# MingyuKim87/Safe_Denoiser

Hardware: AMD Instinct MI355X
Metric: images/sec (512x512, 50 steps, SD-v1.4 + repellency) (higher is better)
Workload: dtype bf16; 1 GPU; README-default end to end (safree = svf = lra = true, safree_neg_prompt_config.json:26-28): token ids -> CLIP -> SAFREE projection -> DDPM 50 steps x UNet on 3 guidance branches with per-prompt text switching + safe_denoiser.yaml repellency (kernel_fast, M=515, sigma 3.15, scale .33, margin 1.6, window 780<=t<=1000) -> VAE decode -> uint8 512x512 images; SD-v1.4 UNet / CLIP / VAE with random weigh; guidance_branches=3, text_encoder_precision=bf16x3, prompts_per_batch=64, latent_repeat=3, renoise_draws_rank0=3520, parallelism=prompt-shard x1

## Files before the change

### safe_denoiser_amd/csrc/sdn_ffn.hip

```cpp
#include "sdn_gemm_common.h"

namespace sdn_gemm_detail {

#define SDN_STAMP(IDX) {}
#ifdef SDN_FFN_STAMPS
__device__ unsigned long long* g_ffn_stamps = nullptr;
#define SDN_FTS_DECL unsigned long long fts_prev = 0, fts_sum[8] = {0, 0, 0, 0, 0, 0, 0, 0};
#define SDN_FTS_MARK(I)                                                                         \
  {                                                                                             \
    unsigned long long t_;                                                                      \
    asm volatile("s_memtime %0\n\ts_waitcnt lgkmcnt(0)" : "=s"(t_)::"memory");                  \
    if ((I) >= 0) fts_sum[(I) < 0 ? 0 : (I)] += t_ - fts_prev;                                  \
    fts_prev = t_;                                                                              \
  }
#define SDN_FTS_FLUSH                                                                           \
  if (g_ffn_stamps && lane == 0)                                                                \
    for (int i_ = 0; i_ < 8; ++i_) g_ffn_stamps[((long)blockIdx.x * 8 + wid) * 8 + i_] = fts_sum[i_];
#else
#define SDN_FTS_DECL
#define SDN_FTS_MARK(I)
#define SDN_FTS_FLUSH
#endif

struct FfnArgs {
  const void* x;
  const float* stats;
  const void* w1;
  const float* c1; const float* d1;
  const void* w2;
  const float* b2;
  const void* residual;
  void* out;
  float* col_stats;
  int M;
};

#define SDN_FFN_CONTRACT(SA, SW)                                                                                           \
      {                                                                                                                    \
        typename T::v8 fa[2][4], fw[2][2];                                                                                 \
        _Pragma("unroll") for (int i = 0; i < 4; ++i)                                                                      \
          fa[0][i] = *reinterpret_cast<const typename T::v8*>((SA) + lds_off(i * 16 + fr, fq));                            \
        _Pragma("unroll") for (int j = 0; j < 2; ++j)                                                                      \
          fw[0][j] = *reinterpret_cast<const typename T::v8*>((SW) + lds_off(j * 16 + fr, fq));                            \
        _Pragma("unroll") for (int gi = 0; gi < 6; ++gi) {                                                                 \
          const int ks = gi / 3, g = gi % 3, nj = g == 2 ? 1 : 2;                                                          \
          if (gi + 1 < 6) {                                                                                                \
            const int ks1 = (gi + 1) / 3, g1 = (gi + 1) % 3, nj1 = g1 == 2 ? 1 : 2;                                        \
            _Pragma("unroll") for (int j = 0; j < nj1; ++j)                                                                \
              fw[(gi + 1) & 1][j] = *reinterpret_cast<const typename T::v8*>((SW) + lds_off((2 * g1 + j) * 16 + fr, ks1 * 4 + fq)); \
          }                                                                                                                \
          if (gi == 1) {                                                                                                   \
            _Pragma("unroll") for (int i = 0; i < 4; ++i)                                                                  \
              fa[1][i] = *reinterpret_cast<const typename T::v8*>((SA) + lds_off(i * 16 + fr, 4 + fq));                    \
          }                                                                                                                \
          __builtin_amdgcn_s_setprio(1);                                                                                   \
          _Pragma("unroll") for (int i = 0; i < 4; ++i)                                                                    \
            _Pragma("unroll") for (int j = 0; j < nj; ++j)                                                                 \
              acc[i][2 * g + j] = T::mfma16(fw[gi & 1][j], fa[ks][i], acc[i][2 * g + j]);                                  \
          __builtin_amdgcn_s_setprio(0);                                                                                   \
        }                                                                                                                  \
      }

template <typename T>
__global__ void __launch_bounds__(512, 1)
k_ffn320(const FfnArgs a) {
#if defined(__HIP_DEVICE_COMPILE__)
  constexpr int C = 320, HID = 4 * C, KT1 = C / BK, NCH = HID / 64, KT2 = NCH + KT1;
  constexpr int BM = 128, BN = C, THREADS = 512, NWAVES = 8, NREP = 5;
  constexpr int XIMG = BM * 128;
  constexpr int W2IMG = C * 128;
  constexpr int OFF_W2A = KT1 * XIMG;
  constexpr int OFF_RING = OFF_W2A + W2IMG;
  constexpr int LDS_BYTES = OFF_RING + W2IMG;
  constexpr unsigned OOB = 0x80000000u;
  __shared__ __attribute__((aligned(1024))) unsigned char smem[LDS_BYTES];

  const int tid = threadIdx.x, lane = tid & 63;
  const int wid = __builtin_amdgcn_readfirstlane(tid >> 6);
  SDN_FTS_DECL
  SDN_FTS_MARK(-1)
  const int wm = wid >> 2, wn = wid & 3;
  const int lrow = lane >> 3, lchunk = (lane & 7) ^ lrow;
  const int fr = lane & 15, fq = lane >> 4;
  const int m0 = blockIdx.x * BM, n0 = 0;

  const __amdgpu_buffer_rsrc_t rs_x = make_rsrc(a.x, (unsigned)((long)a.M * C * 2));
  const __amdgpu_buffer_rsrc_t rs_w1 = make_rsrc(a.w1, (unsigned)(2 * HID * C * 2));
  const __amdgpu_buffer_rsrc_t rs_w2 = make_rsrc(a.w2, (unsigned)(C * (HID + C) * 2));

#pragma unroll
  for (int q = 0; q < 10; ++q) {
    const int p = wid * 10 + q;
    const int kt = p >> 4, rg = p & 15;
    const int m = m0 + rg * 8 + lrow;
    const unsigned off = m < a.M ? (unsigned)(((long)m * C + kt * BK + lchunk * 8) * 2) : OOB;
    __builtin_amdgcn_raw_ptr_buffer_load_lds(rs_x, (lds_ptr_t)(smem + p * 1024), 16, off, 0, 0, 0);
  }
  const unsigned w1_lane = (unsigned)(((wid * 2 * 8 + lrow) * C + lchunk * 8) * 2);
  auto issue_w1 = [&](int g) {
    const int jc = g / KT1, kt = g - jc * KT1;
    unsigned char* dst = smem + OFF_RING + (g & 1) * XIMG + wid * 2048;
    const unsigned base = w1_lane + (unsigned)((jc * 128 * C + kt * BK) * 2);
    __builtin_amdgcn_raw_ptr_buffer_load_lds(rs_w1, (lds_ptr_t)dst, 16, base, 0, 0, 0);
    __builtin_amdgcn_raw_ptr_buffer_load_lds(rs_w1, (lds_ptr_t)(dst + 1024), 16, base + (unsigned)(8 * C * 2), 0, 0, 0);
  };
  const unsigned w2_lane = (unsigned)(((wid * 5 * 8 + lrow) * (HID + C) + lchunk * 8) * 2);
  auto issue_w2_slice = [&](int t, int q, int buf_off) {
    __builtin_amdgcn_raw_ptr_buffer_load_lds(rs_w2, (lds_ptr_t)(smem + buf_off + (wid * 5 + q) * 1024), 16,
                                             w2_lane + (unsigned)((q * 8 * (HID + C) + t * BK) * 2), 0, 0, 0);
  };

  issue_w1(0);
  f32x4 acc[4][NREP];
  {
    f32x4 bv[NREP];
#pragma unroll
    for (int j = 0; j < NREP; ++j) bv[j] = *reinterpret_cast<const f32x4*>(a.b2 + wn * 16 * NREP + j * 16 + fq * 4);
#pragma unroll
    for (int i = 0; i < 4; ++i)
#pragma unroll
      for (int j = 0; j < NREP; ++j) acc[i][j] = bv[j];
  }
  float ln_mu[4] = {0.f, 0.f, 0.f, 0.f}, ln_rs[4] = {0.f, 0.f, 0.f, 0.f};
  const bool own_stats = a.stats == nullptr;
  if (!own_stats) {
#pragma unroll
    for (int i = 0; i < 4; ++i) {
      const int m = m0 + wm * 64 + i * 16 + fr;
      const float2 st2 = *reinterpret_cast<const float2*>(a.stats + 2 * (long)(m < a.M ? m : 0));
      ln_mu[i] = st2.x; ln_rs[i] = st2.y;
    }
  }
  float ln_s1[4] = {0.f, 0.f, 0.f, 0.f}, ln_s2[4] = {0.f, 0.f, 0.f, 0.f};
  f32x4 cv[2], dv[2];
  auto load_cd = [&](int jc) {
#pragma unroll
    for (int j = 0; j < 2; ++j) {
      const int n = jc * 128 + wn * 32 + j * 16 + fq * 4;
      cv[j] = *reinterpret_cast<const f32x4*>(a.c1 + n); dv[j] = *reinterpret_cast<const f32x4*>(a.d1 + n);
    }
  };
  asm volatile("s_waitcnt vmcnt(0)" ::: "memory");
  __syncthreads();

  const unsigned char* sa_x = smem + (wm * 64) * 128;
  SDN_FTS_MARK(0)
  for (int jc = 0; jc < NCH; ++jc) {
    f32x4 acc1[4][2];
#pragma unroll
    for (int i = 0; i < 4; ++i) { acc1[i][0] = (f32x4){0.f, 0.f, 0.f, 0.f}; acc1[i][1] = (f32x4){0.f, 0.f, 0.f, 0.f}; }
#pragma unroll
    for (int kt = 0; kt < KT1; ++kt) {
      const int g = jc * KT1 + kt;
      if (kt == 0) load_cd(jc);
      if (g + 1 < NCH * KT1) issue_w1(g + 1);
      issue_w2_slice(jc, kt, OFF_W2A);
      const unsigned char* sa = sa_x + kt * XIMG;
      const unsigned char* sw = smem + OFF_RING + (g & 1) * XIMG + (wn * 32) * 128;
#pragma unroll
      for (int ks = 0; ks < 2; ++ks) {
        typename T::v8 fa[4], fw[2];
#pragma unroll
        for (int i = 0; i < 4; ++i) fa[i] = *reinterpret_cast<const typename T::v8*>(sa + lds_off(i * 16 + fr, ks * 4 + fq));
#pragma unroll
        for (int j = 0; j < 2; ++j) fw[j] = *reinterpret_cast<const typename T::v8*>(sw + lds_off(j * 16 + fr, ks * 4 + fq));
        if (own_stats && jc == 0) {
#pragma unroll
          for (int i = 0; i < 4; ++i) { ln_s1[i] = T::dot_ones(fa[i], ln_s1[i]); ln_s2[i] = T::dot_self(fa[i], ln_s2[i]); }
        }
        __builtin_amdgcn_s_setprio(1);
#pragma unroll
        for (int i = 0; i < 4; ++i)
#pragma unroll
          for (int j = 0; j < 2; ++j) acc1[i][j] = T::mfma16(fw[j], fa[i], acc1[i][j]);
        __builtin_amdgcn_s_setprio(0);
      }
      SDN_FTS_MARK(1)
      if (kt + 1 < KT1) asm volatile("s_waitcnt vmcnt(1)" ::: "memory");
      else asm volatile("s_waitcnt vmcnt(0)" ::: "memory");
      asm volatile("s_waitcnt lgkmcnt(0)" ::: "memory");
      SDN_FTS_MARK(2)
      __builtin_amdgcn_s_barrier();
      SDN_FTS_MARK(3)
    }
    if (own_stats && jc == 0) {
      const float invk = 1.0f / (float)C;
#pragma unroll
      for (int i = 0; i < 4; ++i) {
        float a1 = ln_s1[i], a2 = ln_s2[i];
        a1 += __shfl_xor(a1, 16, 64); a2 += __shfl_xor(a2, 16, 64);
        a1 += __shfl_xor(a1, 32, 64); a2 += __shfl_xor(a2, 32, 64);
        const float mu = a1 * invk;
        const float var = fmaxf(a2 * invk - mu * mu, 0.f);
        ln_mu[i] = mu; ln_rs[i] = __builtin_amdgcn_rsqf(var + 1e-5f);
      }
    }
    unsigned char* sh = smem + OFF_RING + ((jc * KT1 + KT1 - 1) & 1) * XIMG;
#pragma unroll
    for (int i = 0; i < 4; ++i) {
      const int row = wm * 64 + i * 16 + fr;
      const float mu = ln_mu[i], rs = ln_rs[i];
      const f32x4 hv = (acc1[i][0] - mu * cv[0]) * rs + dv[0], gv = (acc1[i][1] - mu * cv[1]) * rs + dv[1];
      uint2 pk;
      pk.x = T::pack2(hv[0] * gelu_erf(gv[0]), hv[1] * gelu_erf(gv[1]));
      pk.y = T::pack2(hv[2] * gelu_erf(gv[2]), hv[3] * gelu_erf(gv[3]));
      *reinterpret_cast<uint2*>(sh + lds_off(row, wn * 2 + (fq >> 1)) + (fq & 1) * 8) = pk;
    }
    SDN_FTS_MARK(4)
    __syncthreads();
    SDN_FTS_MARK(5)
    {
      const unsigned char* sa = sh + (wm * 64) * 128;
      const unsigned char* sw = smem + OFF_W2A + (wn * 16 * NREP) * 128;
      SDN_FFN_CONTRACT(sa, sw)
    }
    SDN_FTS_MARK(6)
    __syncthreads();
    SDN_FTS_MARK(5)
  }

  const __amdgpu_buffer_rsrc_t rs_res = make_rsrc(a.residual, (unsigned)((long)a.M * C * 2));
  auto issue_residual = [&](int img) {
#pragma unroll
    for (int q = 0; q < 2; ++q) {
      const int piece = img * 16 + wid * 2 + q;
      const int e = piece * 64 + lane;
      const int r = e / (BN / 8), c = e - r * (BN / 8);
      const int m = m0 + r;
      const unsigned off = m < a.M ? (unsigned)(((long)m * C + c * 8) * 2) : OOB;
      __builtin_amdgcn_raw_ptr_buffer_load_lds(rs_res, (lds_ptr_t)(smem + piece * 1024), 16, off, 0, 0, 0);
    }
  };
#pragma unroll
  for (int q = 0; q < 5; ++q) issue_w2_slice(NCH, q, OFF_W2A);
#pragma unroll
  for (int q = 0; q < 5; ++q) issue_w2_slice(NCH + 1, q, OFF_RING);
#pragma unroll
  for (int kt = 0; kt < KT1; ++kt) {
    const int boff = (kt & 1) ? OFF_RING : OFF_W2A;
    if (kt == 0) asm volatile("s_waitcnt vmcnt(5)" ::: "memory");
    else if (kt == 1) asm volatile("s_waitcnt vmcnt(7)" ::: "memory");
    else if (kt == 2 || kt == 3) asm volatile("s_waitcnt vmcnt(9)" ::: "memory");
    else asm volatile("s_waitcnt vmcnt(4)" ::: "memory");
    __builtin_amdgcn_s_barrier();
    {
      const unsigned char* sa = sa_x + kt * XIMG;
      const unsigned char* sw = smem + boff + (wn * 16 * NREP) * 128;
      SDN_FFN_CONTRACT(sa, sw)
    }
    asm volatile("s_waitcnt lgkmcnt(0)" ::: "memory");
    __builtin_amdgcn_s_barrier();
    if (kt + 2 < KT1) {
#pragma unroll
      for (int q = 0; q < 5; ++q) issue_w2_slice(NCH + kt + 2, q, boff);
    }
    issue_residual(kt);
  }
  asm volatile("s_waitcnt vmcnt(0)" ::: "memory");
  __syncthreads();

  GemmArgs g{};
  g.M = a.M; g.N = C; g.K = HID + C; g.ldc = C; g.n_valid = C; g.act = 0; g.out_kind = 0;
  g.residual = (const __bf16*)a.residual; g.out = a.out; g.col_stats = a.col_stats; g.res_lds = 1;
  g.res_bytes = (unsigned)((long)a.M * C * 2); g.rows_per_batch = 0; g.residual_bcast = 0;
  constexpr int LNF = 0, WGM = 2, NSTAGE = 2, STAGE = LDS_BYTES / 2;
  constexpr int CW_PAD = (BN + 8) * 2;
  const bool staged = true;
  const int out_cols = BN;
  const bool res_lds = true;
  const int CW = BN * 2;
  const bool lean = true, lean_gelu = false, lean_gate = false, lean_erf = false;
  constexpr int PASSES = 1, WM_PER_PASS = WGM / PASSES, ROWS_PER_PASS = 64 * WM_PER_PASS;
  static_assert(BM * CW_PAD <= NSTAGE * STAGE - 8 * BN * 8, "staged tile and the column-sum scratch must fit the LDS");
#define SDN_EPI_RES_PRELOADED
#define SDN_PASS 0
#include "sdn_gemm_epilogue.inc"
#undef SDN_PASS
#undef SDN_EPI_RES_PRELOADED
  SDN_FTS_MARK(7)
  SDN_FTS_FLUSH
  (void)NWAVES; (void)WGM; (void)lean_gelu; (void)lean_gate; (void)lean_erf; (void)staged; (void)CW_PAD; (void)KT2;
#endif
}

}
using namespace sdn_gemm_detail;

#ifdef SDN_FFN_STAMPS
extern "C" int sdn_debug_set_ffn_stamps(void* p) { return (int)hipMemcpyToSymbol(HIP_SYMBOL(sdn_gemm_detail::g_ffn_stamps), &p, sizeof(p)); }
#endif
extern "C" int sdn_ffn_geglu_fused(int32_t dtype, int64_t M, int32_t C, const void* x, const float* row_stats, const void* w1_folded, const float* c1,
                        const float* d1, const void* w_cat, const float* b_cat, const void* residual, void* out, float* col_stats,
                        void* stream) {
  auto al16 = [](const void* p) { return (reinterpret_cast<uintptr_t>(p) & 15) == 0; };
  if (dtype < 0 || dtype > 1 || C != 320 || M < 0 || !x || !w1_folded || !c1 || !d1 || !w_cat || !b_cat || !residual || !out)
    return SDN_E_INVALID;
  if (!al16(x) || !al16(w1_folded) || !al16(c1) || !al16(d1) || !al16(w_cat) || !al16(b_cat) || !al16(residual) || !al16(out) ||
      (reinterpret_cast<uintptr_t>(row_stats) & 7) || (reinterpret_cast<uintptr_t>(col_stats) & 7))
    return SDN_E_INVALID;
  if (M * C * 2 >= (1L << 31)) return SDN_E_INVALID;
  if (M == 0) return SDN_OK;
  FfnArgs a{x, row_stats, w1_folded, c1, d1, w_cat, b_cat, residual, out, col_stats, (int)M};
  const unsigned grid = (unsigned)((M + 127) / 128);
  record_gemm_launch(4, dtype, 10, 2, 2, row_stats ? 2 : 1, (int)grid, 1, 1, 0);
  if (dtype == 1) hipLaunchKernelGGL((k_ffn320<SdnF16>), dim3(grid), dim3(512), 0, (hipStream_t)stream, a);
  else hipLaunchKernelGGL((k_ffn320<SdnBF16>), dim3(grid), dim3(512), 0, (hipStream_t)stream, a);
  return sdn_launch_status();
}
```

Before: 8.340 images/sec.

## Stream W1 and W2 chunks through a unified 4-stage LDS ring in fused FFN

New measurement: 8.441 images/sec (median of 6 runs). 1.2% higher.

```diff
diff --git a/safe_denoiser_amd/csrc/sdn_ffn.hip b/safe_denoiser_amd/csrc/sdn_ffn.hip
--- a/safe_denoiser_amd/csrc/sdn_ffn.hip
+++ b/safe_denoiser_amd/csrc/sdn_ffn.hip
@@ -69,9 +69,12 @@
   constexpr int BM = 128, BN = C, THREADS = 512, NWAVES = 8, NREP = 5;
   constexpr int XIMG = BM * 128;
   constexpr int W2IMG = C * 128;
-  constexpr int OFF_W2A = KT1 * XIMG;
-  constexpr int OFF_RING = OFF_W2A + W2IMG;
-  constexpr int LDS_BYTES = OFF_RING + W2IMG;
+  constexpr int NSLOT = 8, NRING = 4;
+  constexpr int OFF_RING = KT1 * XIMG;
+  constexpr int OFF_H = OFF_RING + NRING * XIMG;
+  constexpr int OFF_TA = OFF_RING, OFF_TB = OFF_RING + W2IMG;
+  constexpr int LDS_BYTES = OFF_H + XIMG;
+  static_assert(OFF_TB + W2IMG == LDS_BYTES && NSLOT % NRING == 0, "ring + H = the tail's two weight buffers; stage = slot & 3");
   constexpr unsigned OOB = 0x80000000u;
   __shared__ __attribute__((aligned(1024))) unsigned char smem[LDS_BYTES];
 
@@ -97,12 +100,23 @@
     __builtin_amdgcn_raw_ptr_buffer_load_lds(rs_x, (lds_ptr_t)(smem + p * 1024), 16, off, 0, 0, 0);
   }
   const unsigned w1_lane = (unsigned)(((wid * 2 * 8 + lrow) * C + lchunk * 8) * 2);
-  auto issue_w1 = [&](int g) {
-    const int jc = g / KT1, kt = g - jc * KT1;
-    unsigned char* dst = smem + OFF_RING + (g & 1) * XIMG + wid * 2048;
-    const unsigned base = w1_lane + (unsigned)((jc * 128 * C + kt * BK) * 2);
-    __builtin_amdgcn_raw_ptr_buffer_load_lds(rs_w1, (lds_ptr_t)dst, 16, base, 0, 0, 0);
-    __builtin_amdgcn_raw_ptr_buffer_load_lds(rs_w1, (lds_ptr_t)(dst + 1024), 16, base + (unsigned)(8 * C * 2), 0, 0, 0);
+  const unsigned w2ab_lane = (unsigned)((((wid >> 1) * 16 * NREP + (wid & 1) * 16 + lrow) * (HID + C) + lchunk * 8) * 2);
+  const unsigned w2c_lane = (unsigned)((((wid >> 1) * 16 * NREP + 64 + (wid & 1) * 8 + lrow) * (HID + C) + lchunk * 8) * 2);
+  auto issue_slot = [&](int jc, int u) {
+    if (u >= NSLOT) { u -= NSLOT; ++jc; }
+    if (jc >= NCH) return;
+    unsigned char* stage = smem + OFF_RING + (u & (NRING - 1)) * XIMG;
+    if (u < KT1) {
+      const unsigned base = w1_lane + (unsigned)((jc * 128 * C + u * BK) * 2);
+      __builtin_amdgcn_raw_ptr_buffer_load_lds(rs_w1, (lds_ptr_t)(stage + wid * 2048), 16, base, 0, 0, 0);
+      __builtin_amdgcn_raw_ptr_buffer_load_lds(rs_w1, (lds_ptr_t)(stage + wid * 2048 + 1024), 16, base + (unsigned)(8 * C * 2), 0, 0, 0);
+    } else if (u < NSLOT - 1) {
+      const unsigned base = w2ab_lane + (unsigned)(((u - KT1) * 32 * (HID + C) + jc * BK) * 2);
+      __builtin_amdgcn_raw_ptr_buffer_load_lds(rs_w2, (lds_ptr_t)(stage + wid * 2048), 16, base, 0, 0, 0);
+      __builtin_amdgcn_raw_ptr_buffer_load_lds(rs_w2, (lds_ptr_t)(stage + wid * 2048 + 1024), 16, base + (unsigned)(8 * (HID + C) * 2), 0, 0, 0);
+    } else {
+      __builtin_amdgcn_raw_ptr_buffer_load_lds(rs_w2, (lds_ptr_t)(stage + wid * 1024), 16, w2c_lane + (unsigned)(jc * BK * 2), 0, 0, 0);
+    }
   };
   const unsigned w2_lane = (unsigned)(((wid * 5 * 8 + lrow) * (HID + C) + lchunk * 8) * 2);
   auto issue_w2_slice = [&](int t, int q, int buf_off) {
@@ -110,7 +124,7 @@
                                              w2_lane + (unsigned)((q * 8 * (HID + C) + t * BK) * 2), 0, 0, 0);
   };
 
-  issue_w1(0);
+  issue_slot(0, 0); issue_slot(0, 1); issue_slot(0, 2);
   f32x4 acc[4][NREP];
   {
     f32x4 bv[NREP];
@@ -146,17 +160,16 @@
   const unsigned char* sa_x = smem + (wm * 64) * 128;
   SDN_FTS_MARK(0)
   for (int jc = 0; jc < NCH; ++jc) {
+    const bool last = jc == NCH - 1;
     f32x4 acc1[4][2];
 #pragma unroll
     for (int i = 0; i < 4; ++i) { acc1[i][0] = (f32x4){0.f, 0.f, 0.f, 0.f}; acc1[i][1] = (f32x4){0.f, 0.f, 0.f, 0.f}; }
 #pragma unroll
     for (int kt = 0; kt < KT1; ++kt) {
-      const int g = jc * KT1 + kt;
       if (kt == 0) load_cd(jc);
-      if (g + 1 < NCH * KT1) issue_w1(g + 1);
-      issue_w2_slice(jc, kt, OFF_W2A);
+      issue_slot(jc, kt + 3);
       const unsigned char* sa = sa_x + kt * XIMG;
-      const unsigned char* sw = smem + OFF_RING + (g & 1) * XIMG + (wn * 32) * 128;
+      const unsigned char* sw = smem + OFF_RING + (kt & (NRING - 1)) * XIMG + (wn * 32) * 128;
 #pragma unroll
       for (int ks = 0; ks < 2; ++ks) {
         typename T::v8 fa[4], fw[2];
@@ -176,13 +189,15 @@
         __builtin_amdgcn_s_setprio(0);
       }
       SDN_FTS_MARK(1)
-      if (kt + 1 < KT1) asm volatile("s_waitcnt vmcnt(1)" ::: "memory");
-      else asm volatile("s_waitcnt vmcnt(0)" ::: "memory");
+      if (kt == 0) asm volatile("s_waitcnt vmcnt(8)" ::: "memory");
+      else if (kt < KT1 - 1) asm volatile("s_waitcnt vmcnt(4)" ::: "memory");
+      else asm volatile("s_waitcnt vmcnt(3)" ::: "memory");
       asm volatile("s_waitcnt lgkmcnt(0)" ::: "memory");
       SDN_FTS_MARK(2)
       __builtin_amdgcn_s_barrier();
       SDN_FTS_MARK(3)
     }
+    issue_slot(jc, KT1 + 3);
     if (own_stats && jc == 0) {
       const float invk = 1.0f / (float)C;
 #pragma unroll
@@ -195,7 +210,8 @@
         ln_mu[i] = mu; ln_rs[i] = __builtin_amdgcn_rsqf(var + 1e-5f);
       }
     }
-    unsigned char* sh = smem + OFF_RING + ((jc * KT1 + KT1 - 1) & 1) * XIMG;
+    unsigned char* sh = smem + OFF_H;
+    unsigned h_addr = 0;
 #pragma unroll
     for (int i = 0; i < 4; ++i) {
       const int row = wm * 64 + i * 16 + fr;
@@ -204,19 +220,48 @@
       uint2 pk;
       pk.x = T::pack2(hv[0] * gelu_erf(gv[0]), hv[1] * gelu_erf(gv[1]));
       pk.y = T::pack2(hv[2] * gelu_erf(gv[2]), hv[3] * gelu_erf(gv[3]));
-      *reinterpret_cast<uint2*>(sh + lds_off(row, wn * 2 + (fq >> 1)) + (fq & 1) * 8) = pk;
-    }
+      if (i == 0) h_addr = (unsigned)(unsigned long)(lds_ptr_t)(sh + lds_off(row, wn * 2 + (fq >> 1)) + (fq & 1) * 8);
+      asm volatile("ds_write_b64 %0, %1 offset:%2" ::"v"(h_addr), "v"((unsigned long long)pk.y << 32 | pk.x), "i"(i * 16 * 128) : "memory");
+    }
+    asm volatile("s_waitcnt lgkmcnt(0)" ::: "memory");
     SDN_FTS_MARK(4)
-    __syncthreads();
+    __builtin_amdgcn_s_barrier();
+    asm volatile("" ::: "memory");
     SDN_FTS_MARK(5)
     {
-      const unsigned char* sa = sh + (wm * 64) * 128;
-      const unsigned char* sw = smem + OFF_W2A + (wn * 16 * NREP) * 128;
-      SDN_FFN_CONTRACT(sa, sw)
-    }
-    SDN_FTS_MARK(6)
-    __syncthreads();
-    SDN_FTS_MARK(5)
+      typename T::v8 fa[2][4];
+#pragma unroll
+      for (int ks = 0; ks < 2; ++ks)
+#pragma unroll
+        for (int i = 0; i < 4; ++i)
+          fa[ks][i] = *reinterpret_cast<const typename T::v8*>(sh + (wm * 64) * 128 + lds_off(i * 16 + fr, ks * 4 + fq));
+#pragma unroll
+      for (int v = 0; v < 3; ++v) {
+        const int u = KT1 + v, nj = v == 2 ? 1 : 2;
+        if (v > 0) issue_slot(jc, u + 3);
+        const unsigned char* sw = smem + OFF_RING + (u & (NRING - 1)) * XIMG + (wn * 16 * nj) * 128;
+        typename T::v8 fw[2][2];
+#pragma unroll
+        for (int ks = 0; ks < 2; ++ks)
+#pragma unroll
+          for (int j = 0; j < nj; ++j) fw[ks][j] = *reinterpret_cast<const typename T::v8*>(sw + lds_off(j * 16 + fr, ks * 4 + fq));
+        __builtin_amdgcn_s_setprio(1);
+#pragma unroll
+        for (int ks = 0; ks < 2; ++ks)
+#pragma unroll
+          for (int i = 0; i < 4; ++i)
+#pragma unroll
+            for (int j = 0; j < nj; ++j) acc[i][2 * v + j] = T::mfma16(fw[ks][j], fa[ks][i], acc[i][2 * v + j]);
+        __builtin_amdgcn_s_setprio(0);
+        SDN_FTS_MARK(6)
+        if (last) asm volatile("s_waitcnt vmcnt(0)" ::: "memory");
+        else if (v == 0) asm volatile("s_waitcnt vmcnt(3)" ::: "memory");
+        else asm volatile("s_waitcnt vmcnt(4)" ::: "memory");
+        asm volatile("s_waitcnt lgkmcnt(0)" ::: "memory");
+        __builtin_amdgcn_s_barrier();
+        SDN_FTS_MARK(5)
+      }
+    }
   }
 
   const __amdgpu_buffer_rsrc_t rs_res = make_rsrc(a.residual, (unsigned)((long)a.M * C * 2));
@@ -232,12 +277,12 @@
     }
   };
 #pragma unroll
-  for (int q = 0; q < 5; ++q) issue_w2_slice(NCH, q, OFF_W2A);
-#pragma unroll
-  for (int q = 0; q < 5; ++q) issue_w2_slice(NCH + 1, q, OFF_RING);
+  for (int q = 0; q < 5; ++q) issue_w2_slice(NCH, q, OFF_TA);
+#pragma unroll
+  for (int q = 0; q < 5; ++q) issue_w2_slice(NCH + 1, q, OFF_TB);
 #pragma unroll
   for (int kt = 0; kt < KT1; ++kt) {
-    const int boff = (kt & 1) ? OFF_RING : OFF_W2A;
+    const int boff = (kt & 1) ? OFF_TB : OFF_TA;
     if (kt == 0) asm volatile("s_waitcnt vmcnt(5)" ::: "memory");
     else if (kt == 1) asm volatile("s_waitcnt vmcnt(7)" ::: "memory");
     else if (kt == 2 || kt == 3) asm volatile("s_waitcnt vmcnt(9)" ::: "memory");
```
